# tsurumeso/vocal-remover

Measured on NVIDIA H100. Metric: seconds-of-audio/sec separated (n_fft=2048, hop=1024), higher is better.
Workload: dtype bf16x3 (split-bf16 operands hi+lo, 3 wgmma passes, fp32 accumulate); fft/lstm fp32

## Files before the change

vocal-remover_b200/csrc/api.cu:

```cuda
#include <stdio.h>
#include <string.h>

#include <string>

#include "../../include/vr_b200.h"
#include "engine.h"
#include "kernels.h"
#include "tc_plan.h"

struct vr_ctx {
  vr::Engine* eng;
  std::string err;
};

static std::string g_create_err;

static int fail(vr_ctx* c, const std::string& m) {
  (c ? c->err : g_create_err) = m;
  return -1;
}
static void use_device(const vr_ctx* c) {
  if (c && c->eng) cudaSetDevice(c->eng->cfg().device);
}
static int done(vr_ctx* c, bool ok) {
// ... 259 lines not shown
int vr_flac_encode_analyse(vr_ctx* ctx, const float* x, int32_t channels, int64_t n, int32_t rate_code, int32_t bits,
                           void* pcm, int32_t* plan, void* stream) {
  use_device(ctx);
  return cuda_result(ctx, "vr_flac_encode_analyse",
                     vr::launch_flac_encode_analyse(x, channels, n, rate_code, bits, pcm, plan, (cudaStream_t)stream));
}

int vr_flac_encode_pack(vr_ctx* ctx, const void* pcm, int32_t channels, int64_t n, int32_t bits, const int32_t* plan,
                        const int64_t* offsets, int32_t rate_code, int32_t rate_value, uint8_t* out, int32_t* status,
                        void* stream) {
  use_device(ctx);
  return cuda_result(ctx, "vr_flac_encode_pack",
                     vr::launch_flac_encode_pack(pcm, channels, n, bits, plan, offsets, rate_code, rate_value, out,
                                                 status, (cudaStream_t)stream));
}

int vr_pcm_pack(vr_ctx* ctx, const float* x, int32_t channels, int64_t n, int32_t bits, uint8_t* out, void* stream) {
  use_device(ctx);
  return cuda_result(ctx, "vr_pcm_pack", vr::launch_pcm_pack(x, channels, n, bits, out, (cudaStream_t)stream));
}

static int64_t bss_workspace(bool framewise, int32_t K, int32_t C, int64_t N, int32_t L, int64_t window, int64_t hop,
                             int32_t frames_per_batch) {
  std::string err;
  const int64_t bytes = vr::bss_eval_workspace(framewise, K, C, N, L, window, hop, frames_per_batch, err);
  if (bytes < 0) fail(nullptr, err);
  return bytes;
}

static int bss_run(vr_ctx* ctx, bool framewise, const float* refs, const float* ests, int32_t K, int32_t C, int64_t N,
                   int32_t L, int64_t window, int64_t hop, int32_t frames_per_batch, void* workspace,
                   int64_t workspace_bytes, double* frames_host, double* corr_host, double* loading_host,
                   double* phase_ms, void* stream) {
  use_device(ctx);
  std::string err;
  return vr::bss_eval(framewise, refs, ests, K, C, N, L, window, hop, frames_per_batch, workspace, workspace_bytes,
                      frames_host, corr_host, loading_host, phase_ms, (cudaStream_t)stream, err)
             ? 0
             : fail(ctx, err);
}

int64_t vr_bss_eval_workspace(int32_t K, int32_t C, int64_t N, int32_t L, int64_t window, int64_t hop) {
  return bss_workspace(false, K, C, N, L, window, hop, 1);
}

int vr_bss_eval(vr_ctx* ctx, const float* refs, const float* ests, int32_t K, int32_t C, int64_t N, int32_t L,
                int64_t window, int64_t hop, void* workspace, int64_t workspace_bytes, double* frames_host,
                double* corr_host, double* loading_host, double* phase_ms, void* stream) {
  return bss_run(ctx, false, refs, ests, K, C, N, L, window, hop, 1, workspace, workspace_bytes, frames_host,
                 corr_host, loading_host, phase_ms, stream);
}

int64_t vr_bss_eval_framewise_workspace(int32_t K, int32_t C, int64_t N, int32_t L, int64_t window, int64_t hop,
                                        int32_t frames_per_batch) {
  return bss_workspace(true, K, C, N, L, window, hop, frames_per_batch);
}

int vr_bss_eval_framewise(vr_ctx* ctx, const float* refs, const float* ests, int32_t K, int32_t C, int64_t N,
                          int32_t L, int64_t window, int64_t hop, int32_t frames_per_batch, void* workspace,
                          int64_t workspace_bytes, double* frames_host, double* corr_host, double* loading_host,
                          double* phase_ms, void* stream) {
  return bss_run(ctx, true, refs, ests, K, C, N, L, window, hop, frames_per_batch, workspace, workspace_bytes,
                 frames_host, corr_host, loading_host, phase_ms, stream);
}

int vr_shared_alloc(vr_ctx* ctx, int64_t bytes, void** dev_ptr, unsigned char* handle64) {
  CHECK_CTX(ctx);
  if (!dev_ptr || !handle64 || bytes <= 0) return fail(ctx, "vr_shared_alloc: bad arguments");
  static_assert(sizeof(cudaIpcMemHandle_t) == 64, "CUDA IPC handle is 64 bytes");
  void* p = nullptr;
  cudaError_t e = cudaMalloc(&p, (size_t)bytes);
  if (e != cudaSuccess) return fail(ctx, std::string("vr_shared_alloc: cudaMalloc: ") + cudaGetErrorString(e));
  cudaIpcMemHandle_t h;
  e = cudaIpcGetMemHandle(&h, p);
  if (e != cudaSuccess) {
    cudaFree(p);
    return fail(ctx, std::string("vr_shared_alloc: cudaIpcGetMemHandle: ") + cudaGetErrorString(e));
  }
  memcpy(handle64, &h, 64);
  *dev_ptr = p;
  return 0;
}

int vr_shared_open(vr_ctx* ctx, const unsigned char* handle64, void** dev_ptr) {
  CHECK_CTX(ctx);
  if (!dev_ptr || !handle64) return fail(ctx, "vr_shared_open: bad arguments");
  cudaIpcMemHandle_t h;
  memcpy(&h, handle64, 64);
  void* p = nullptr;
  cudaError_t e = cudaIpcOpenMemHandle(&p, h, cudaIpcMemLazyEnablePeerAccess);
  if (e != cudaSuccess) return fail(ctx, std::string("vr_shared_open: cudaIpcOpenMemHandle: ") + cudaGetErrorString(e));
  *dev_ptr = p;
  return 0;
}

int vr_shared_close(vr_ctx* ctx, void* dev_ptr, int32_t owner) {
  CHECK_CTX(ctx);
  if (!dev_ptr) return 0;
  cudaError_t e = owner ? cudaFree(dev_ptr) : cudaIpcCloseMemHandle(dev_ptr);
  if (e != cudaSuccess) return fail(ctx, std::string("vr_shared_close: ") + cudaGetErrorString(e));
  return 0;
}

int64_t vr_launch_count(const vr_ctx* ctx) { return ctx && ctx->eng ? ctx->eng->launches : 0; }

int vr_profile_enable(vr_ctx* ctx, int32_t on) {
  CHECK_CTX(ctx);
  ctx->eng->profile_enable(on != 0);
  return 0;
}

int vr_profile_read(vr_ctx* ctx, double* out6) {
  CHECK_CTX(ctx);
  return done(ctx, ctx->eng->profile_read(out6));
}

int vr_profile_dump(vr_ctx* ctx, char* text, int64_t cap, int64_t* needed) {
  CHECK_CTX(ctx);
  std::string t;
  if (!ctx->eng->profile_dump(t)) return done(ctx, false);
  if (needed) *needed = (int64_t)t.size() + 1;
  if (text && cap > 0) {
    const size_t n = t.size() < (size_t)cap - 1 ? t.size() : (size_t)cap - 1;
    memcpy(text, t.data(), n);
    text[n] = 0;
  }
  return 0;
}

int vr_debug_conv(vr_ctx* ctx, const float* x, int32_t N, int32_t Cin, int32_t H, int32_t W, const float* w,
                  const float* bias, int32_t Cout, int32_t k, int32_t stride, int32_t dil_h, int32_t dil_w, int32_t act,
                  int32_t use_tc, float* y, void* stream) {
  CHECK_CTX(ctx);
  return done(ctx, ctx->eng->debug_conv(x, N, Cin, H, W, w, bias, Cout, k, stride, dil_h, dil_w, act, use_tc, y,
                                        (cudaStream_t)stream));
}

int vr_debug_decoder(vr_ctx* ctx, const float* low, int32_t N, int32_t Cl, int32_t h, int32_t w, const float* skip,
                     int32_t Cs, const float* wgt, const float* bias, int32_t Cout, int32_t act, int32_t fused, float* y,
                     void* stream) {
  CHECK_CTX(ctx);
  return done(ctx, ctx->eng->debug_decoder(low, N, Cl, h, w, skip, Cs, wgt, bias, Cout, act, fused, y,
                                           (cudaStream_t)stream));
}

int vr_debug_tensor(vr_ctx* ctx, const char* name, int32_t n0, int32_t n, float* out, int64_t* shape4, void* stream) {
  CHECK_NET(ctx);
  if (!name || !shape4) return fail(ctx, "vr_debug_tensor: name and shape4 are required");
  return done(ctx, ctx->eng->debug_tensor(name, n0, n, out, shape4, (cudaStream_t)stream));
}

int vr_debug_set(int32_t key, int32_t value) {
  int* knob = key == 0 ? &vr::g_debug.trace : key == 2 ? &vr::g_debug.rows_wide : key == 3 ? &vr::g_debug.halo
            : key == 6 ? &vr::g_debug.kskip : key == 7 ? &vr::g_debug.crop_mask : nullptr;
  if (!knob) return -1;
  *knob = value;
  return 0;
}

int64_t vr_debug_trace(uint64_t* host_out, int64_t capacity) {
  return vr::tc_rows_read_trace((unsigned long long*)host_out, (long long)capacity);
}

}
```

vocal-remover_b200/csrc/conv_tc.cu:

```cuda
#include <cuda.h>
#include <stdio.h>

#include <map>
#include <tuple>

#include "engine.h"
#include "tc_common.cuh"
#include "tc_plan.h"

namespace vr {

static constexpr int kMaxStages = 8;
static constexpr int kConsumerWarps = 8;
static constexpr int kThreads = 32 * kConsumerWarps + 32;
static constexpr int kStaticSmem = 2048;

struct TcParams {
  int N, Ho, Wo, Wt, Ht, Nt, tiles_w, tiles_h, m_tiles, n_tiles;
  int stride, pad_h, pad_w, dil_h, dil_w, KW;
  int cchunks, total_sub, CinPadTC, Cout, act, stages;
  bf16* out_hi;
  bf16* out_lo;
  int64_t osn, osh;
  int osw;
  const float* bias;
};

template <int KB, int BN>
__global__ void __launch_bounds__(kThreads, 1)
    conv_tc_kernel(const __grid_constant__ CUtensorMap tmA, const __grid_constant__ CUtensorMap tmB, const TcParams p) {
  constexpr int SUBS = 64 / KB;
  constexpr int kSteps = KB / 16;
  constexpr uint32_t kAPlane = 128 * KB * 2;
  constexpr uint32_t kASub = 2 * kAPlane;
  constexpr uint32_t kBPlane = BN * KB * 2;
  constexpr uint32_t kBSub = 2 * kBPlane;
  constexpr uint32_t kStageBytes = SUBS * (kASub + kBSub);
  constexpr uint32_t kBRegion = SUBS * kASub;
  constexpr uint32_t kLayout = KB == 64 ? 1u : KB == 32 ? 2u : 3u;
  extern __shared__ uint8_t smem_raw[];
  __shared__ __align__(8) uint64_t bar_full[kMaxStages];
  __shared__ __align__(8) uint64_t bar_empty[kMaxStages];
  __shared__ float bias_s[256];

  const int warp = __shfl_sync(0xffffffffu, (int)threadIdx.x >> 5, 0);
  const int lane = threadIdx.x & 31;
  const uint32_t smem_base = (smem_u32(smem_raw) + 1023u) & ~1023u;
  const int total_tiles = p.m_tiles * p.n_tiles;
  const int num_iters = (p.total_sub + SUBS - 1) / SUBS;

  if (warp == kConsumerWarps && lane == 0) {
    tma_prefetch(&tmA);
    tma_prefetch(&tmB);
    MbarRing(smem_u32(&bar_full[0]), smem_u32(&bar_empty[0]), 0, p.stages).init(1, kConsumerWarps);
    asm volatile("fence.mbarrier_init.release.cluster;" ::: "memory");
  }
  for (int i = threadIdx.x; i < p.n_tiles * BN; i += blockDim.x) bias_s[i] = __ldg(p.bias + i);
  __syncthreads();

  if (warp == kConsumerWarps) {
    if (elect_one_sync()) {
      MbarRing ring(smem_u32(&bar_full[0]), smem_u32(&bar_empty[0]), 0, p.stages);
      for (int tile = blockIdx.x; tile < total_tiles; tile += gridDim.x) {
        const int nt = tile % p.n_tiles;
        const int mt = tile / p.n_tiles;
        const int w0 = (mt % p.tiles_w) * p.Wt;
        const int h0 = ((mt / p.tiles_w) % p.tiles_h) * p.Ht;
        const int n0 = (mt / (p.tiles_w * p.tiles_h)) * p.Nt;
        const int wbase = w0 * p.stride - p.pad_w, hbase = h0 * p.stride - p.pad_h;
        const int nrow = nt * BN;
        int cc = 0, kw = 0, kh = 0, sub = 0;
        for (int it = 0; it < num_iters; ++it) {
          ring.wait_empty();
          const int nsub = min(SUBS, p.total_sub - sub);
          const uint32_t full = ring.full();
          const uint32_t sbase = smem_base + (uint32_t)ring.slot * kStageBytes;
          mbar_expect_tx(full, (uint32_t)nsub * (kASub + kBSub));
#pragma unroll
          for (int j = 0; j < SUBS; ++j) {
            if (j < nsub) {
              tma_load_5d(sbase + (uint32_t)j * kASub, &tmA, cc * KB, wbase + kw * p.dil_w, hbase + kh * p.dil_h, n0, 0, full);
              tma_load_3d(sbase + kBRegion + (uint32_t)j * kBSub, &tmB, (kh * p.KW + kw) * p.CinPadTC + cc * KB, nrow, 0,
                          full);
              ++sub;
              if (++cc == p.cchunks) {
                cc = 0;
                if (++kw == p.KW) {
                  kw = 0;
                  ++kh;
                }
              }
            }
          }
          ring.advance();
        }
      }
    }
    __syncwarp();
  } else {
    const int wg = warp >> 2;
    const float slope = act_slope(p.act);
    const uint32_t dhi = desc_hi(8 * KB * 2, kLayout);
    MbarRing ring(smem_u32(&bar_full[0]), smem_u32(&bar_empty[0]), 0, p.stages);
    float acc[BN / 2];
    for (int tile = blockIdx.x; tile < total_tiles; tile += gridDim.x) {
#pragma unroll
      for (int i = 0; i < BN / 2; ++i) acc[i] = 0.f;
      HeldSlot held;
      for (int it = 0; it < num_iters; ++it) {
        const int nsub = min(SUBS, p.total_sub - it * SUBS);
        ring.wait_full();
        const uint32_t sdesc = desc_lo(smem_base + (uint32_t)ring.slot * kStageBytes);
        wg_fence();
#pragma unroll
        for (int j = 0; j < SUBS; ++j) {
          if (j < nsub) {
            const uint32_t a_hi = sdesc + ((j * kASub + (uint32_t)wg * (kAPlane / 2)) >> 4);
            const uint32_t a_lo = a_hi + (kAPlane >> 4);
            const uint32_t b_hi = sdesc + ((kBRegion + j * kBSub) >> 4);
            const uint32_t b_lo = b_hi + (kBPlane >> 4);
#pragma unroll
            for (int k = 0; k < kSteps; ++k)
              wgmma_split3<BN>(acc, a_hi + 2u * k, a_lo + 2u * k, b_hi + 2u * k, b_lo + 2u * k, dhi);
          }
        }
        wg_commit();
        wg_wait<1>();
        held.release(ring, lane);
        held.hold(ring);
        ring.advance();
      }
      wg_wait<0>();
      held.release_last(ring, lane);

      const int nt = tile % p.n_tiles;
      const int mt = tile / p.n_tiles;
      const int w0 = (mt % p.tiles_w) * p.Wt;
      const int h0 = ((mt / p.tiles_w) % p.tiles_h) * p.Ht;
      const int n0 = (mt / (p.tiles_w * p.tiles_h)) * p.Nt;
      const int c_lane = nt * BN + 2 * (lane & 3);
#pragma unroll
      for (int hr = 0; hr < 2; ++hr) {
        const int row = 64 * wg + 16 * (warp & 3) + (lane >> 2) + 8 * hr;
        const int dw = row % p.Wt;
        const int dh = (row / p.Wt) % p.Ht;
        const int n = n0 + row / (p.Wt * p.Ht);
        if (n >= p.N) continue;
        const int64_t obase = (int64_t)n * p.osn + (int64_t)(h0 + dh) * p.osh + (int64_t)(w0 + dw) * p.osw;
#pragma unroll
        for (int j = 0; j < BN / 8; ++j)
          epilogue_pair(acc[4 * j + 2 * hr], acc[4 * j + 2 * hr + 1], bias_s, c_lane + 8 * j, p.Cout, slope,
                        p.out_hi + obase, p.out_lo + obase);
      }
    }
  }
}

#define VR_TC_FOR_BN(X, KB) X(KB, 16) X(KB, 32) X(KB, 48) X(KB, 64) X(KB, 80) X(KB, 96) X(KB, 112) X(KB, 128)
#define VR_TC_FOR_ALL(X) VR_TC_FOR_BN(X, 64) VR_TC_FOR_BN(X, 32) VR_TC_FOR_BN(X, 16)


TcDebug g_debug;

static constexpr int kMaxDevices = 64;
const TcDevice& tc_device() {
  static TcDevice table[kMaxDevices];
  static TcDevice none;
  int dev = -1;
  if (cudaGetDevice(&dev) != cudaSuccess || dev < 0 || dev >= kMaxDevices) return none;
  TcDevice& d = table[dev];
  if (!d.ok) {
    if (cudaDeviceGetAttribute(&d.max_smem, cudaDevAttrMaxSharedMemoryPerBlockOptin, dev) != cudaSuccess ||
        cudaDeviceGetAttribute(&d.num_sms, cudaDevAttrMultiProcessorCount, dev) != cudaSuccess)
      return none;
#define VR_TC_SET_SMEM(KB, BN) \
  cudaFuncSetAttribute(conv_tc_kernel<KB, BN>, cudaFuncAttributeMaxDynamicSharedMemorySize, d.max_smem - kStaticSmem);
    VR_TC_FOR_ALL(VR_TC_SET_SMEM)
#undef VR_TC_SET_SMEM
    tc_rows_set_attributes(d.max_smem);
    tc_halo_set_attributes(d.max_smem);
    d.ok = true;
  }
  return d;
}

typedef CUresult (*EncodeTiledFn)(CUtensorMap*, CUtensorMapDataType, cuuint32_t, void*, const cuuint64_t*,
                                  const cuuint64_t*, const cuuint32_t*, const cuuint32_t*, CUtensorMapInterleave,
                                  CUtensorMapSwizzle, CUtensorMapL2promotion, CUtensorMapFloatOOBfill);
static EncodeTiledFn tc_encode_fn() {
  static EncodeTiledFn fn = nullptr;
  if (!fn) {
    void* p = nullptr;
    cudaDriverEntryPointQueryResult q;
    if (cudaGetDriverEntryPoint("cuTensorMapEncodeTiled", &p, cudaEnableDefault, &q) == cudaSuccess &&
        q == cudaDriverEntryPointSuccess)
      fn = (EncodeTiledFn)p;
  }
  return fn;
}

static CUtensorMapSwizzle swizzle_for(int KB) {
  return KB == 64 ? CU_TENSOR_MAP_SWIZZLE_128B : KB == 32 ? CU_TENSOR_MAP_SWIZZLE_64B : CU_TENSOR_MAP_SWIZZLE_32B;
}

static uint16_t tc_f2bf(float f) {
  uint32_t u;
  memcpy(&u, &f, 4);
  if ((u & 0x7fffffffu) > 0x7f800000u) return (uint16_t)((u >> 16) | 0x40);
  uint32_t r = 0x7fffu + ((u >> 16) & 1u);
  return (uint16_t)((u + r) >> 16);
}
static float tc_bf2f(uint16_t h) {
  uint32_t u = (uint32_t)h << 16;
  float f;
  memcpy(&f, &u, 4);
  return f;
}

struct TileGeom {
  int Wt, Ht, Nt;
  bool ok;
};
static TileGeom tile_geom(int Ho, int Wo) {
  TileGeom g{0, 0, 0, false};
  if (Wo <= 0 || Ho <= 0) return g;
  if (Wo >= 128) {
    if (Wo % 128) return g;
    g.Wt = 128; g.Ht = 1; g.Nt = 1;
  } else {
    if (128 % Wo) return g;
    g.Wt = Wo;
    g.Ht = 128 / Wo < Ho ? 128 / Wo : Ho;
    if (Ho % g.Ht) return g;
    if ((128 / Wo) % g.Ht) return g;
    g.Nt = 128 / (g.Wt * g.Ht);
  }
  g.ok = true;
  return g;
}

struct NTiling {
  int BN, n_tiles;
};
static NTiling n_tiling(const ConvLayer& L, bool rows, bool rows_wide) {
  const int cout16 = round_up(L.Cout, 16);
  if (rows) {
    const int BN = cout16 == 16 ? 16 : (rows_wide && cout16 % 64 == 0 ? 64 : 32);
    return {BN, ceil_div(cout16, BN)};
  }
  const int n_tiles = ceil_div(cout16, 128);
  return {round_up(ceil_div(cout16, n_tiles), 16), n_tiles};
}

TcKind tc_choose(const ConvLayer& L, int H, int W, bool rows_wide) {
  if (!(L.k == 1 || L.k == 3) || !(L.stride == 1 || L.stride == 2) || L.Cout < 4) return TC_NONE;
  const TileGeom g = tile_geom(H, W);
  if (!g.ok || g.Wt * L.stride > 256 || g.Ht * L.stride > 256) return TC_NONE;
  const bool k3s1 = L.k == 3 && L.stride == 1 && L.dil_h == 1 && L.dil_w == 1;
  const NTiling r = n_tiling(L, true, rows_wide), t = n_tiling(L, false, false);
  if (k3s1 && W % 128 == 0 && H % 8 == 0 && tc_rows_has(r.BN) && r.n_tiles * r.BN <= 256) return TC_ROWS;
  if (k3s1 && (W == 16 || W == 32 || W == 64) && H % (128 / W) == 0 && tc_halo_has(t.BN) &&
      t.n_tiles * t.BN <= 256 && g_debug.halo != 1)
    return TC_HALO;
  if (t.n_tiles * t.BN > 256) return TC_NONE;
  return TC_GENERIC;
}

template <class At>
static std::vector<uint16_t> split_bf16(const ConvLayer& L, const float* wp, int rows, int K, At at) {
  std::vector<uint16_t> planes((size_t)2 * rows * K, 0);
  const size_t lo = (size_t)rows * K;
  for (int co = 0; co < L.Cout; ++co)
    for (int t = 0; t < L.k * L.k; ++t)
      for (int ci = 0; ci < L.CinPad; ++ci) {
        const float w = wp[((size_t)t * L.CinPad + ci) * L.CoutPad + co];
        const uint16_t hi = tc_f2bf(w);
        const size_t i = at(co, t, ci);
        planes[i] = hi;
        planes[lo + i] = tc_f2bf(w - tc_bf2f(hi));
      }
  return planes;
}

static unsigned long long weight_group_mask(const ConvLayer& L, const float* wp, int CinPad) {
  if (CinPad / 8 > 64) return ~0ull;
  unsigned long long m = 0x3ull;
  for (int ci = 0; ci < L.CinPad; ++ci) {
    bool any = false;
    for (int t = 0; t < L.k * L.k && !any; ++t)
      for (int co = 0; co < L.Cout && !any; ++co) any = wp[((size_t)t * L.CinPad + ci) * L.CoutPad + co] != 0.f;
    if (any) m |= 1ull << (ci / 8);
  }
  return m;
}

static bool encode_weight_map(TcConv& tc, int rows, int K, int box_rows, std::string& err, const std::string& name) {
  cuuint64_t dims[3] = {(cuuint64_t)K, (cuuint64_t)rows, 2};
  cuuint64_t strides[2] = {(cuuint64_t)K * 2, (cuuint64_t)rows * K * 2};
  cuuint32_t box[3] = {(cuuint32_t)tc.KB, (cuuint32_t)box_rows, 2};
  cuuint32_t es[3] = {1, 1, 1};
  CUresult r = tc_encode_fn()(&tc.map_b, CU_TENSOR_MAP_DATA_TYPE_BFLOAT16, 3, tc.w_planes.get(), dims, strides, box, es,
                              CU_TENSOR_MAP_INTERLEAVE_NONE, swizzle_for(tc.KB), CU_TENSOR_MAP_L2_PROMOTION_L2_256B,
                              CU_TENSOR_MAP_FLOAT_OOB_FILL_NONE);
  if (r != CUDA_SUCCESS) {
    err = "cuTensorMapEncodeTiled(weights) failed for " + name + " code " + std::to_string((int)r);
    return false;
  }
  return true;
}

const CUtensorMap* tc_activation_map(TcConv& tc, const ActView& v, int bw, int bh, int bn, int es, std::string& err,
                                     const std::string& name) {
  const ViewKey key = std::make_tuple((const void*)v.hi, (const void*)v.lo, v.N, v.H, v.W, v.C, bw, bh, bn);
  auto it = tc.map_a.find(key);
  if (it != tc.map_a.end()) return &it->second;
  const int64_t plane = (const char*)v.lo - (const char*)v.hi;
  if (v.sw % 8 || v.sh % 8 || v.sn % 8 || (reinterpret_cast<uintptr_t>(v.hi) & 15) || plane <= 0 || plane % 16) {
    err = "internal: the input of " + name + " is not 16-byte aligned or its lo plane does not follow its hi plane";
    return nullptr;
  }
  cuuint64_t dims[5] = {(cuuint64_t)v.C, (cuuint64_t)v.W, (cuuint64_t)v.H, (cuuint64_t)v.N, 2};
  cuuint64_t strides[4] = {(cuuint64_t)v.sw * 2, (cuuint64_t)v.sh * 2, (cuuint64_t)v.sn * 2, (cuuint64_t)plane};
  cuuint32_t box[5] = {(cuuint32_t)tc.KB, (cuuint32_t)bw, (cuuint32_t)bh, (cuuint32_t)bn, 2};
  cuuint32_t estr[5] = {1, (cuuint32_t)es, (cuuint32_t)es, 1, 1};
  CUtensorMap m;
  CUresult r = tc_encode_fn()(&m, CU_TENSOR_MAP_DATA_TYPE_BFLOAT16, 5, (void*)v.hi, dims, strides, box, estr,
                              CU_TENSOR_MAP_INTERLEAVE_NONE, swizzle_for(tc.KB), CU_TENSOR_MAP_L2_PROMOTION_L2_256B,
                              CU_TENSOR_MAP_FLOAT_OOB_FILL_NONE);
  if (r != CUDA_SUCCESS) {
    err = "cuTensorMapEncodeTiled(activations) failed for " + name + " code " + std::to_string((int)r);
    return nullptr;
  }
  return &tc.map_a.emplace(key, m).first->second;
}

bool tc_prepare(ConvLayer& L, const float* w, const float* b, int H, int W, bool rows_wide, std::string& err) {
  const TcKind kind = tc_choose(L, H, W, rows_wide);
  if (kind == TC_NONE) return true;
  if (!tc_encode_fn()) {
    err = "cuTensorMapEncodeTiled is not available from the driver";
    return false;
  }
  auto tc = std::make_shared<TcConv>();
  tc->kind = kind;
  tc->H = H; tc->W = W;
  const NTiling nt = n_tiling(L, kind == TC_ROWS, rows_wide);
  const int BN = nt.BN, cin16 = round_up(L.CinPad, 16);
  tc->BN = BN; tc->n_tiles = nt.n_tiles;
  tc->KB = kind != TC_GENERIC ? 32 : cin16 % 64 == 0 ? 64 : cin16 % 32 == 0 ? 32 : 16;
  const int CinPad = round_up(L.CinPad, tc->KB);
  tc->CinPad = CinPad;
  tc->chunks = CinPad / tc->KB;
  tc->kmask = weight_group_mask(L, w, CinPad);
  const int rows = nt.n_tiles * BN;
  std::vector<uint16_t> planes;
  int brows, K;
  if (kind == TC_ROWS) {
    brows = 3 * rows;
    K = 3 * CinPad;
    planes = split_bf16(L, w, brows, K, [&](int co, int t, int ci) {
      return (size_t)(co / BN * 3 * BN + (2 - t / 3) * BN + co % BN) * K + (size_t)(t % 3) * CinPad + ci;
    });
  } else {
    brows = rows;
    K = L.k * L.k * CinPad;
    planes = split_bf16(L, w, brows, K, [&](int co, int t, int ci) { return (size_t)co * K + (size_t)t * CinPad + ci; });
  }
  std::vector<float> bias((size_t)rows, 0.f);
  for (int co = 0; co < L.Cout; ++co) bias[(size_t)co] = b[co];
  if (tc->w_planes.alloc(planes.size() * 2) != cudaSuccess || tc->bias.alloc(bias.size() * 4) != cudaSuccess) {
    err = "cudaMalloc failed while packing tensor-core weights for " + L.name;
    return false;
  }
  if (!upload(tc->w_planes.get(), planes.data(), planes.size() * 2, err) ||
      !upload(tc->bias.get(), bias.data(), bias.size() * 4, err) ||
      !encode_weight_map(*tc, brows, K, kind == TC_ROWS ? 3 * BN : BN, err, L.name))
    return false;
  L.tc = tc;
  return true;
}

cudaError_t tc_launch(const ConvLayer& L, const ActView& in, const ActView& out, cudaStream_t s, std::string& err,
                      const ConvFusion& f) {
  TcConv& tc = *L.tc;
  if (out.H != tc.H || out.W != tc.W || (in.H - 1) / L.stride + 1 != out.H || (in.W - 1) / L.stride + 1 != out.W) {
    err = "internal: " + L.name + " is launched on maps of another size than it was prepared for";
    return cudaErrorInvalidValue;
  }
  if (tc.kind == TC_ROWS) return tc_rows_launch(L, tc, in, out, s, err, f);
  if (!f.empty()) {
    err = "tc_launch: fused work is only implemented in the row-streaming kernel";
    return cudaErrorInvalidValue;
  }
  if (tc.kind == TC_HALO) return tc_halo_launch(L, tc, in, out, s, err);
  const TileGeom g = tile_geom(out.H, out.W);
  const CUtensorMap* map_a = tc_activation_map(tc, in, g.Wt * L.stride, g.Ht * L.stride, g.Nt, L.stride, err, L.name);
  if (!map_a) return cudaErrorInvalidValue;
  const int SUBS = 64 / tc.KB;
  TcParams p;
  p.N = out.N; p.Ho = out.H; p.Wo = out.W;
  p.Wt = g.Wt; p.Ht = g.Ht; p.Nt = g.Nt;
  p.tiles_w = out.W / g.Wt; p.tiles_h = out.H / g.Ht;
  p.m_tiles = p.tiles_w * p.tiles_h * ceil_div(out.N, g.Nt);
  p.n_tiles = tc.n_tiles;
  p.stride = L.stride; p.dil_h = L.dil_h; p.dil_w = L.dil_w;
  p.pad_h = L.dil_h * (L.k / 2); p.pad_w = L.dil_w * (L.k / 2);
  p.KW = L.k;
  p.cchunks = tc.chunks; p.total_sub = L.k * L.k * tc.chunks;
  p.CinPadTC = tc.CinPad; p.Cout = L.Cout; p.act = L.act;
  const int stage_bytes = SUBS * (2 * 128 * tc.KB * 2 + 2 * tc.BN * tc.KB * 2);
  const TcDevice& dv = tc_device();
  if (!dv.ok) {
    err = "tc_launch: cannot query the current device";
    return cudaErrorInvalidValue;
  }
  const int dyn = dv.max_smem - kStaticSmem;
  p.stages = (dyn - 1024) / stage_bytes;
  if (p.stages > kMaxStages) p.stages = kMaxStages;
  if (p.stages < 2) {
    err = "tc_launch: shared memory too small for two pipeline stages";
    return cudaErrorInvalidValue;
  }
  p.out_hi = out.hi; p.out_lo = out.lo;
  p.osn = out.sn; p.osh = out.sh; p.osw = out.sw;
  p.bias = tc.bias.get();
  const int total_tiles = p.m_tiles * p.n_tiles;
  const int grid = total_tiles < dv.num_sms ? total_tiles : dv.num_sms;
#define VR_TC_LAUNCH(KB_, BN_)                                                       \
  if (tc.KB == KB_ && tc.BN == BN_) {                                                \
    conv_tc_kernel<KB_, BN_><<<grid, kThreads, dyn, s>>>(*map_a, tc.map_b, p);       \
    return cudaGetLastError();                                                       \
  }
  VR_TC_FOR_ALL(VR_TC_LAUNCH)
#undef VR_TC_LAUNCH
  err = "tc_launch: no kernel instantiation for this channel tile";
  return cudaErrorInvalidValue;
}

}
```

vocal-remover_b200/csrc/tc_plan.h:

```cpp
#pragma once
#include <cuda.h>

#include <map>
#include <tuple>

#include "engine.h"

namespace vr {

enum TcKind {
  TC_NONE,
  TC_GENERIC,
  TC_ROWS,
  TC_HALO,
};

typedef std::tuple<const void*, const void*, int, int, int, int, int, int, int> ViewKey;

struct TcConv {
  TcKind kind = TC_NONE;
  int H = 0, W = 0;
  int KB = 0, CinPad = 0, chunks = 0, BN = 0, n_tiles = 0;
  unsigned long long kmask = ~0ull;
  DevPtr<bf16> w_planes;
  DevPtr<float> bias;
  CUtensorMap map_b;
  std::map<ViewKey, CUtensorMap> map_a;
  bool fuses_upsample(int up_C) const { return kind == TC_ROWS && up_C % 32 == 0 && up_C <= CinPad; }
  bool fuses_dot() const { return kind == TC_ROWS; }
  bool fuses_mask(int Cout, int offset, bool up) const {
    const int kept = W - 2 * offset;
    return kind == TC_ROWS && up && n_tiles == 1 && BN <= 32 && BN == Cout && offset >= 0 && kept > 0 &&
           kept % 128 == 0;
  }
};

TcKind tc_choose(const ConvLayer& L, int H, int W, bool rows_wide);
const CUtensorMap* tc_activation_map(TcConv& tc, const ActView& v, int bw, int bh, int bn, int es, std::string& err,
                                     const std::string& name);

cudaError_t tc_rows_launch(const ConvLayer& L, TcConv& tc, const ActView& in, const ActView& out, cudaStream_t s,
                           std::string& err, const ConvFusion& f);
void tc_rows_set_attributes(int max_smem);
bool tc_rows_has(int BN);
int tc_rows_read_trace(unsigned long long* out, long long capacity);

cudaError_t tc_halo_launch(const ConvLayer& L, TcConv& tc, const ActView& in, const ActView& out, cudaStream_t s,
                           std::string& err);
void tc_halo_set_attributes(int max_smem);
bool tc_halo_has(int BN);

struct TcDevice {
  bool ok = false;
  int num_sms = 0, max_smem = 0;
};
const TcDevice& tc_device();

struct TcDebug {
  int trace = 0;
  int rows_wide = 0;
  int halo = 0;
  int kskip = 1;
  int crop_mask = 1;
};
extern TcDebug g_debug;

}
```

Before: 2902.

## Pair M or N tiles per CTA in generic TC conv to share operand loads

Adds PAIR_M and PAIR_N modes to the generic tensor-core conv kernel. In these modes one CTA runs 16 consumer warps over two M tiles that share a B tile, or two N tiles that share an A tile, with a smaller K stage. A heuristic picks pairing only for small KB/BN layers, and only when it cuts the number of SM waves roughly in half. The goal is to reduce redundant operand traffic and wave quantization on small layers. The epilogue also gains vectorized 16-byte stores, at the cost of more template instantiations, extra tensor maps and higher register pressure.

```diff
diff --git a/profiles/generic_conv.py b/profiles/generic_conv.py
--- /dev/null
+++ b/profiles/generic_conv.py
@@ -0,0 +1,171 @@
+import argparse
+import ctypes
+import json
+import os
+import statistics
+import subprocess
+import sys
+
+ROOT = os.path.dirname(os.path.dirname(os.path.abspath(__file__)))
+PKG = os.path.join(ROOT, 'vocal-remover_b200')
+for p in (ROOT, PKG):
+    if p not in sys.path:
+        sys.path.insert(0, p)
+
+NETS = [('stg1_low', 16, 512), ('stg1_high', 8, 512), ('stg2_low', 32, 512), ('stg2_high', 16, 512),
+        ('stg3_full', 32, 1024)]
+W = 256
+NOUT = 32
+
+
+def generic_layers():
+    out = {}
+    mult = [1, 2, 4, 6, 8]
+    for net, n, H in NETS:
+        for i in range(4):
+            key = (n * mult[i], H >> i, W >> i, n * mult[i + 1], 3, 2, 1, 1, 2)
+            out.setdefault(key, []).append('%s.enc%d.conv1' % (net, i + 2))
+        c8, h16, w16 = 8 * n, H // 16, W // 16
+        out.setdefault((c8, 1, w16, c8, 1, 1, 1, 1, 1), []).append(net + '.aspp.conv1.1')
+        out.setdefault((c8, h16, w16, c8, 1, 1, 1, 1, 1), []).append(net + '.aspp.conv2')
+        for j, (dh, dw) in enumerate([(4, 2), (8, 4), (12, 6)]):
+            out.setdefault((c8, h16, w16, c8, 3, 1, dh, dw, 1), []).append('%s.aspp.conv%d' % (net, j + 3))
+        out.setdefault((5 * c8, h16, w16, c8, 1, 1, 1, 1, 1), []).append(net + '.aspp.bottleneck')
+    out.setdefault((NOUT // 2, 512, W, NOUT // 4, 1, 1, 1, 1, 1), []).append('stg1_low_band_net.1')
+    out.setdefault((NOUT, 512, W, NOUT // 2, 1, 1, 1, 1, 1), []).append('stg2_low_band_net.1')
+    return out
+
+
+def _ceil(a, b):
+    return -(-a // b)
+
+
+def tiling(N, g):
+    Cin, H, Wi, Cout, k, s = g[:6]
+    Ho, Wo = (H - 1) // s + 1, (Wi - 1) // s + 1
+    cout16 = _ceil(Cout, 16) * 16
+    n_tiles = _ceil(cout16, 128)
+    BN = _ceil(_ceil(cout16, n_tiles), 16) * 16
+    cin16 = _ceil(Cin, 16) * 16
+    if Wo >= 128:
+        Wt, Ht, Nt = 128, 1, 1
+    else:
+        Wt, Ht = Wo, min(128 // Wo, Ho)
+        Nt = 128 // (Wt * Ht)
+    m_tiles = (Wo // Wt) * (Ho // Ht) * _ceil(N, Nt)
+    KB = 64 if cin16 % 64 == 0 else 32 if cin16 % 32 == 0 else 16
+    return dict(Ho=Ho, Wo=Wo, BN=BN, n_tiles=n_tiles, m_tiles=m_tiles, CinPad=cin16, KB=KB,
+                flops=2.0 * N * Ho * Wo * Cout * Cin * k * k)
+
+
+def operand_bytes(t, k, mode):
+    per = k * k * t['CinPad'] * 4
+    m, nt, BN = t['m_tiles'], t['n_tiles'], t['BN']
+    if mode == 'PAIR_M':
+        return per * nt * (128 * m + BN * _ceil(m, 2))
+    if mode == 'PAIR_N':
+        return per * m * (128 + 2 * BN)
+    return per * m * nt * (128 + BN)
+
+
+def auto_mode(t, num_sms):
+    if t['KB'] > 32 or t['BN'] > 32:
+        return 'NONE'
+    pair = 'PAIR_N' if t['n_tiles'] == 2 and t['KB'] >= 32 else 'PAIR_M'
+    units = t['m_tiles'] if pair == 'PAIR_N' else _ceil(t['m_tiles'], 2) * t['n_tiles']
+    w1, w2 = _ceil(t['m_tiles'] * t['n_tiles'], num_sms), _ceil(units, num_sms)
+    return pair if 19 * w2 <= 10 * w1 else 'NONE'
+
+
+def _gpu_info():
+    try:
+        r = subprocess.run(['nvidia-smi', '--query-gpu=name,power.limit,clocks.max.sm,clocks.sm',
+                            '--format=csv,noheader'], capture_output=True, text=True, timeout=30)
+        name, power, max_clock, clock = [s.strip() for s in r.stdout.splitlines()[0].split(',')]
+        return dict(gpu=name, power_limit=power, max_sm_clock=max_clock, sm_clock=clock)
+    except Exception as e:
+        return dict(gpu=None, nvidia_smi_error=str(e))
+
+
+def _run_conv(ctx, x, w, b, g):
+    import torch
+    from lib import _native
+    Cin, H, Wi, Cout, k, s, dh, dw, act = g
+    N = x.shape[0]
+    Ho, Wo = (H - 1) // s + 1, (Wi - 1) // s + 1
+    y = torch.empty((N, Cout, Ho, Wo), dtype=torch.float32, device='cuda')
+    ctx.check(ctx.lib.vr_debug_conv(ctx.handle, _native.ptr(x), N, Cin, H, Wi, _native.ptr(w), _native.ptr(b), Cout,
+                                    k, s, dh, dw, act, 1, _native.ptr(y), _native.stream_ptr()), 'vr_debug_conv')
+
+
+def _profiled_ms(ctx):
+    need = ctypes.c_int64(0)
+    ctx.check(ctx.lib.vr_profile_dump(ctx.handle, None, 0, ctypes.byref(need)), 'vr_profile_dump')
+    buf = ctypes.create_string_buffer(need.value)
+    ctx.check(ctx.lib.vr_profile_dump(ctx.handle, buf, need.value, None), 'vr_profile_dump')
+    return [float(ln.split()[5]) for ln in buf.value.decode().splitlines() if ln.split()[0] == 'debug_conv']
+
+
+def main():
+    ap = argparse.ArgumentParser()
+    ap.add_argument('--batch', type=int, default=27)
+    ap.add_argument('--runs', type=int, default=10)
+    ap.add_argument('--warmup', type=int, default=3)
+    ap.add_argument('--out', type=str, default='')
+    args = ap.parse_args()
+    import torch
+    from lib import _native
+    assert torch.cuda.is_available(), 'generic_conv.py times the GPU kernels: it needs a CUDA device'
+    info = _gpu_info()
+    info['torch_device'] = torch.cuda.get_device_name(0)
+    num_sms = torch.cuda.get_device_properties(0).multi_processor_count
+    ctx = _native.Context(0, 2048, 1024, NOUT, 128, 256, 1, 0)
+    modes = [(1, 'NONE'), (2, 'PAIR_M'), (3, 'PAIR_N'), (0, 'auto')]
+    rows = []
+    N = args.batch
+    print('# %s, power limit %s, max SM clock %s (SM clock %s at start); batch %d, median of %d launches'
+          % (info.get('gpu') or info['torch_device'], info.get('power_limit'), info.get('max_sm_clock'),
+             info.get('sm_clock'), N, args.runs))
+    print('%-28s %-38s %5s %5s %6s  %-8s %8s %7s %8s' % ('layers', 'Cin,H,W,Cout,k,s,dh,dw', 'BN', 'nt', 'mt', 'key',
+                                                         'ms', 'TFLOP/s', 'B/FLOP'))
+    try:
+        for gi, (g, names) in enumerate(generic_layers().items()):
+            Cin, H, Wi, Cout, k = g[:5]
+            t = tiling(N, g)
+            gen = torch.Generator().manual_seed(gi)
+            x = torch.randn(N, Cin, H, Wi, generator=gen).cuda()
+            w = (torch.randn(Cout, Cin, k, k, generator=gen) / (Cin * k * k) ** 0.5).cuda()
+            b = (torch.randn(Cout, generator=gen) * 0.1).cuda()
+            auto = auto_mode(t, num_sms)
+            for key, mode in modes:
+                if mode == 'PAIR_N' and not (t['n_tiles'] == 2 and t['KB'] >= 32):
+                    continue
+                ctx.lib.vr_debug_set(8, key)
+                for _ in range(args.warmup):
+                    _run_conv(ctx, x, w, b, g)
+                ctx.check(ctx.lib.vr_profile_enable(ctx.handle, 1), 'vr_profile_enable')
+                for _ in range(args.runs):
+                    _run_conv(ctx, x, w, b, g)
+                ms = statistics.median(_profiled_ms(ctx))
+                ctx.check(ctx.lib.vr_profile_enable(ctx.handle, 0), 'vr_profile_enable')
+                ran = auto if mode == 'auto' else mode
+                bpf = operand_bytes(t, k, ran) / t['flops']
+                row = dict(layers=names, geometry=list(g), batch=N, key=key, mode=ran, ms=ms,
+                           tflops=t['flops'] / ms * 1e-9, operand_bytes_per_flop=bpf, **t)
+                rows.append(row)
+                print('%-28s %-38s %5d %5d %6d  %-8s %8.4f %7.1f %8.4f' % (
+                    names[0] + ('' if len(names) == 1 else ' +%d' % (len(names) - 1)), ','.join(map(str, g[:8])),
+                    t['BN'], t['n_tiles'], t['m_tiles'], '%d %s' % (key, ran if key == 0 else ''), ms,
+                    row['tflops'], bpf))
+    finally:
+        ctx.lib.vr_debug_set(8, 0)
+        ctx.close()
+    info_end = _gpu_info()
+    print('# SM clock at end: %s' % info_end.get('sm_clock'))
+    if args.out:
+        with open(args.out, 'w') as f:
+            json.dump(dict(gpu=info, sm_clock_end=info_end.get('sm_clock'), rows=rows), f, indent=1)
+
+
+if __name__ == '__main__':
+    main()
diff --git a/vocal-remover_b200/csrc/api.cu b/vocal-remover_b200/csrc/api.cu
--- a/vocal-remover_b200/csrc/api.cu
+++ b/vocal-remover_b200/csrc/api.cu
@@ -435,7 +435,8 @@
 
 int vr_debug_set(int32_t key, int32_t value) {
   int* knob = key == 0 ? &vr::g_debug.trace : key == 2 ? &vr::g_debug.rows_wide : key == 3 ? &vr::g_debug.halo
-            : key == 6 ? &vr::g_debug.kskip : key == 7 ? &vr::g_debug.crop_mask : nullptr;
+            : key == 6 ? &vr::g_debug.kskip : key == 7 ? &vr::g_debug.crop_mask
+            : key == 8 ? &vr::g_debug.pair : nullptr;
   if (!knob) return -1;
   *knob = value;
   return 0;
diff --git a/vocal-remover_b200/csrc/conv_tc.cu b/vocal-remover_b200/csrc/conv_tc.cu
--- a/vocal-remover_b200/csrc/conv_tc.cu
+++ b/vocal-remover_b200/csrc/conv_tc.cu
@@ -11,8 +11,9 @@
 namespace vr {
 
 static constexpr int kMaxStages = 8;
-static constexpr int kConsumerWarps = 8;
-static constexpr int kThreads = 32 * kConsumerWarps + 32;
+__host__ __device__ constexpr int consumer_warps(int mode) { return mode == PAIR_NONE ? 8 : 16; }
+__host__ __device__ constexpr int tc_threads(int mode) { return 32 * consumer_warps(mode) + 32; }
+__host__ __device__ constexpr int stage_k(int mode) { return mode == PAIR_NONE ? 64 : 32; }
 static constexpr int kStaticSmem = 2048;
 
 struct TcParams {
@@ -24,19 +25,33 @@
   int64_t osn, osh;
   int osw;
   const float* bias;
+  int vec16;
 };
 
-template <int KB, int BN>
-__global__ void __launch_bounds__(kThreads, 1)
+__device__ __forceinline__ void act_split2(float v0, float v1, const float* bias_s, int c, float slope, uint32_t& hi,
+                                           uint32_t& lo) {
+  const float t0 = v0 + bias_s[c], t1 = v1 + bias_s[c + 1];
+  const float y0 = fmaxf(t0, 0.f) + slope * fminf(t0, 0.f);
+  const float y1 = fmaxf(t1, 0.f) + slope * fminf(t1, 0.f);
+  hi = f2_to_bf2(y0, y1);
+  const float2 hf = bf2_to_f2(hi);
+  lo = f2_to_bf2(y0 - hf.x, y1 - hf.y);
+}
+
+template <int KB, int BN, int MODE>
+__global__ void __launch_bounds__(tc_threads(MODE), 1)
     conv_tc_kernel(const __grid_constant__ CUtensorMap tmA, const __grid_constant__ CUtensorMap tmB, const TcParams p) {
-  constexpr int SUBS = 64 / KB;
+  constexpr int kConsumerWarps = consumer_warps(MODE);
+  constexpr int SUBS = stage_k(MODE) / KB;
+  constexpr int NA = MODE == PAIR_M ? 2 : 1;
+  constexpr int NB = MODE == PAIR_N ? 2 : 1;
   constexpr int kSteps = KB / 16;
   constexpr uint32_t kAPlane = 128 * KB * 2;
   constexpr uint32_t kASub = 2 * kAPlane;
   constexpr uint32_t kBPlane = BN * KB * 2;
   constexpr uint32_t kBSub = 2 * kBPlane;
-  constexpr uint32_t kStageBytes = SUBS * (kASub + kBSub);
-  constexpr uint32_t kBRegion = SUBS * kASub;
+  constexpr uint32_t kStageBytes = SUBS * (NA * kASub + NB * kBSub);
+  constexpr uint32_t kBRegion = SUBS * NA * kASub;
   constexpr uint32_t kLayout = KB == 64 ? 1u : KB == 32 ? 2u : 3u;
   extern __shared__ uint8_t smem_raw[];
   __shared__ __align__(8) uint64_t bar_full[kMaxStages];
@@ -46,7 +61,8 @@
   const int warp = __shfl_sync(0xffffffffu, (int)threadIdx.x >> 5, 0);
   const int lane = threadIdx.x & 31;
   const uint32_t smem_base = (smem_u32(smem_raw) + 1023u) & ~1023u;
-  const int total_tiles = p.m_tiles * p.n_tiles;
+  const int n_units = p.n_tiles / NB;
+  const int total_units = (p.m_tiles + NA - 1) / NA * n_units;
   const int num_iters = (p.total_sub + SUBS - 1) / SUBS;
 
   if (warp == kConsumerWarps && lane == 0) {
@@ -61,27 +77,37 @@
   if (warp == kConsumerWarps) {
     if (elect_one_sync()) {
       MbarRing ring(smem_u32(&bar_full[0]), smem_u32(&bar_empty[0]), 0, p.stages);
-      for (int tile = blockIdx.x; tile < total_tiles; tile += gridDim.x) {
-        const int nt = tile % p.n_tiles;
-        const int mt = tile / p.n_tiles;
-        const int w0 = (mt % p.tiles_w) * p.Wt;
-        const int h0 = ((mt / p.tiles_w) % p.tiles_h) * p.Ht;
-        const int n0 = (mt / (p.tiles_w * p.tiles_h)) * p.Nt;
-        const int wbase = w0 * p.stride - p.pad_w, hbase = h0 * p.stride - p.pad_h;
-        const int nrow = nt * BN;
+      for (int unit = blockIdx.x; unit < total_units; unit += gridDim.x) {
+        const int nt0 = unit % n_units * NB;
+        const int mt0 = unit / n_units * NA;
+        const int na = min(NA, p.m_tiles - mt0);
+        int wbase[NA], hbase[NA], n0[NA];
+#pragma unroll
+        for (int a = 0; a < NA; ++a) {
+          const int mt = mt0 + a;
+          wbase[a] = (mt % p.tiles_w) * p.Wt * p.stride - p.pad_w;
+          hbase[a] = ((mt / p.tiles_w) % p.tiles_h) * p.Ht * p.stride - p.pad_h;
+          n0[a] = (mt / (p.tiles_w * p.tiles_h)) * p.Nt;
+        }
         int cc = 0, kw = 0, kh = 0, sub = 0;
         for (int it = 0; it < num_iters; ++it) {
           ring.wait_empty();
           const int nsub = min(SUBS, p.total_sub - sub);
           const uint32_t full = ring.full();
           const uint32_t sbase = smem_base + (uint32_t)ring.slot * kStageBytes;
-          mbar_expect_tx(full, (uint32_t)nsub * (kASub + kBSub));
+          mbar_expect_tx(full, (uint32_t)nsub * ((uint32_t)na * kASub + NB * kBSub));
 #pragma unroll
           for (int j = 0; j < SUBS; ++j) {
             if (j < nsub) {
-              tma_load_5d(sbase + (uint32_t)j * kASub, &tmA, cc * KB, wbase + kw * p.dil_w, hbase + kh * p.dil_h, n0, 0, full);
-              tma_load_3d(sbase + kBRegion + (uint32_t)j * kBSub, &tmB, (kh * p.KW + kw) * p.CinPadTC + cc * KB, nrow, 0,
-                          full);
+#pragma unroll
+              for (int a = 0; a < NA; ++a)
+                if (a < na)
+                  tma_load_5d(sbase + (uint32_t)(j * NA + a) * kASub, &tmA, cc * KB, wbase[a] + kw * p.dil_w,
+                              hbase[a] + kh * p.dil_h, n0[a], 0, full);
+#pragma unroll
+              for (int b = 0; b < NB; ++b)
+                tma_load_3d(sbase + kBRegion + (uint32_t)(j * NB + b) * kBSub, &tmB,
+                            (kh * p.KW + kw) * p.CinPadTC + cc * KB, (nt0 + b) * BN, 0, full);
               ++sub;
               if (++cc == p.cchunks) {
                 cc = 0;
@@ -98,12 +124,24 @@
     }
     __syncwarp();
   } else {
-    const int wg = warp >> 2;
+    const int half = (warp >> 2) & 1;
+    const int pair = warp >> 3;
+    const int a_sel = MODE == PAIR_M ? pair : 0, b_sel = MODE == PAIR_N ? pair : 0;
     const float slope = act_slope(p.act);
     const uint32_t dhi = desc_hi(8 * KB * 2, kLayout);
     MbarRing ring(smem_u32(&bar_full[0]), smem_u32(&bar_empty[0]), 0, p.stages);
     float acc[BN / 2];
-    for (int tile = blockIdx.x; tile < total_tiles; tile += gridDim.x) {
+    for (int unit = blockIdx.x; unit < total_units; unit += gridDim.x) {
+      const int nt = unit % n_units * NB + b_sel;
+      const int mt = unit / n_units * NA + a_sel;
+      if (mt >= p.m_tiles) {
+        for (int it = 0; it < num_iters; ++it) {
+          ring.wait_full();
+          warp_arrive(ring.empty(), lane);
+          ring.advance();
+        }
+        continue;
+      }
 #pragma unroll
       for (int i = 0; i < BN / 2; ++i) acc[i] = 0.f;
       HeldSlot held;
@@ -115,9 +153,9 @@
 #pragma unroll
         for (int j = 0; j < SUBS; ++j) {
           if (j < nsub) {
-            const uint32_t a_hi = sdesc + ((j * kASub + (uint32_t)wg * (kAPlane / 2)) >> 4);
+            const uint32_t a_hi = sdesc + (((j * NA + a_sel) * kASub + (uint32_t)half * (kAPlane / 2)) >> 4);
             const uint32_t a_lo = a_hi + (kAPlane >> 4);
-            const uint32_t b_hi = sdesc + ((kBRegion + j * kBSub) >> 4);
+            const uint32_t b_hi = sdesc + ((kBRegion + (j * NB + b_sel) * kBSub) >> 4);
             const uint32_t b_lo = b_hi + (kBPlane >> 4);
 #pragma unroll
             for (int k = 0; k < kSteps; ++k)
@@ -133,31 +171,72 @@
       wg_wait<0>();
       held.release_last(ring, lane);
 
-      const int nt = tile % p.n_tiles;
-      const int mt = tile / p.n_tiles;
       const int w0 = (mt % p.tiles_w) * p.Wt;
       const int h0 = ((mt / p.tiles_w) % p.tiles_h) * p.Ht;
       const int n0 = (mt / (p.tiles_w * p.tiles_h)) * p.Nt;
-      const int c_lane = nt * BN + 2 * (lane & 3);
+      const int q = lane & 3;
+      const int c_lane = nt * BN + 2 * q;
 #pragma unroll
       for (int hr = 0; hr < 2; ++hr) {
-        const int row = 64 * wg + 16 * (warp & 3) + (lane >> 2) + 8 * hr;
+        const int row = 64 * half + 16 * (warp & 3) + (lane >> 2) + 8 * hr;
         const int dw = row % p.Wt;
         const int dh = (row / p.Wt) % p.Ht;
         const int n = n0 + row / (p.Wt * p.Ht);
-        if (n >= p.N) continue;
         const int64_t obase = (int64_t)n * p.osn + (int64_t)(h0 + dh) * p.osh + (int64_t)(w0 + dw) * p.osw;
-#pragma unroll
-        for (int j = 0; j < BN / 8; ++j)
-          epilogue_pair(acc[4 * j + 2 * hr], acc[4 * j + 2 * hr + 1], bias_s, c_lane + 8 * j, p.Cout, slope,
-                        p.out_hi + obase, p.out_lo + obase);
+        if constexpr (BN % 32 == 0 && (MODE == PAIR_NONE || BN <= 64)) {
+          const bool keep = n < p.N;
+#pragma unroll
+          for (int jb = 0; jb < BN / 8; jb += 4) {
+            if (p.vec16 && nt * BN + 8 * (jb + 4) <= p.Cout) {
+              uint32_t hi[4], lo[4], oh[4], ol[4];
+#pragma unroll
+              for (int g = 0; g < 4; ++g)
+                act_split2(acc[4 * (jb + g) + 2 * hr], acc[4 * (jb + g) + 2 * hr + 1], bias_s, c_lane + 8 * (jb + g),
+                           slope, hi[g], lo[g]);
+#pragma unroll
+              for (int s = 0; s < 4; ++s) {
+                const int gs = (q + s) & 3, src = (q - s) & 3;
+                const uint32_t sh = gs == 0 ? hi[0] : gs == 1 ? hi[1] : gs == 2 ? hi[2] : hi[3];
+                const uint32_t sl = gs == 0 ? lo[0] : gs == 1 ? lo[1] : gs == 2 ? lo[2] : lo[3];
+                const uint32_t rh = __shfl_sync(0xffffffffu, sh, (lane & ~3) | src);
+                const uint32_t rl = __shfl_sync(0xffffffffu, sl, (lane & ~3) | src);
+#pragma unroll
+                for (int g = 0; g < 4; ++g)
+                  if (src == g) {
+                    oh[g] = rh;
+                    ol[g] = rl;
+                  }
+              }
+              if (keep) {
+                const int c = nt * BN + 8 * (jb + q);
+                *reinterpret_cast<uint4*>(p.out_hi + obase + c) = make_uint4(oh[0], oh[1], oh[2], oh[3]);
+                *reinterpret_cast<uint4*>(p.out_lo + obase + c) = make_uint4(ol[0], ol[1], ol[2], ol[3]);
+              }
+            } else if (keep) {
+#pragma unroll
+              for (int j = jb; j < jb + 4; ++j)
+                epilogue_pair(acc[4 * j + 2 * hr], acc[4 * j + 2 * hr + 1], bias_s, c_lane + 8 * j, p.Cout, slope,
+                              p.out_hi + obase, p.out_lo + obase);
+            }
+          }
+        } else {
+          if (n >= p.N) continue;
+#pragma unroll
+          for (int j = 0; j < BN / 8; ++j)
+            epilogue_pair(acc[4 * j + 2 * hr], acc[4 * j + 2 * hr + 1], bias_s, c_lane + 8 * j, p.Cout, slope,
+                          p.out_hi + obase, p.out_lo + obase);
+        }
       }
     }
   }
 }
 
-#define VR_TC_FOR_BN(X, KB) X(KB, 16) X(KB, 32) X(KB, 48) X(KB, 64) X(KB, 80) X(KB, 96) X(KB, 112) X(KB, 128)
-#define VR_TC_FOR_ALL(X) VR_TC_FOR_BN(X, 64) VR_TC_FOR_BN(X, 32) VR_TC_FOR_BN(X, 16)
+#define VR_TC_FOR_BN(X, KB, M) \
+  X(KB, 16, M) X(KB, 32, M) X(KB, 48, M) X(KB, 64, M) X(KB, 80, M) X(KB, 96, M) X(KB, 112, M) X(KB, 128, M)
+#define VR_TC_FOR_ALL(X)                                                                                   \
+  VR_TC_FOR_BN(X, 64, PAIR_NONE) VR_TC_FOR_BN(X, 32, PAIR_NONE) VR_TC_FOR_BN(X, 16, PAIR_NONE)             \
+  VR_TC_FOR_BN(X, 32, PAIR_M) VR_TC_FOR_BN(X, 16, PAIR_M)                                                  \
+  X(32, 80, PAIR_N) X(32, 96, PAIR_N) X(32, 112, PAIR_N) X(32, 128, PAIR_N)
 
 
 TcDebug g_debug;
@@ -173,8 +252,8 @@
     if (cudaDeviceGetAttribute(&d.max_smem, cudaDevAttrMaxSharedMemoryPerBlockOptin, dev) != cudaSuccess ||
         cudaDeviceGetAttribute(&d.num_sms, cudaDevAttrMultiProcessorCount, dev) != cudaSuccess)
       return none;
-#define VR_TC_SET_SMEM(KB, BN) \
-  cudaFuncSetAttribute(conv_tc_kernel<KB, BN>, cudaFuncAttributeMaxDynamicSharedMemorySize, d.max_smem - kStaticSmem);
+#define VR_TC_SET_SMEM(KB, BN, M) \
+  cudaFuncSetAttribute(conv_tc_kernel<KB, BN, M>, cudaFuncAttributeMaxDynamicSharedMemorySize, d.max_smem - kStaticSmem);
     VR_TC_FOR_ALL(VR_TC_SET_SMEM)
 #undef VR_TC_SET_SMEM
     tc_rows_set_attributes(d.max_smem);
@@ -294,13 +373,14 @@
   return m;
 }
 
-static bool encode_weight_map(TcConv& tc, int rows, int K, int box_rows, std::string& err, const std::string& name) {
+static bool encode_weight_map(const TcConv& tc, CUtensorMap* map, int kb, int rows, int K, int box_rows,
+                              std::string& err, const std::string& name) {
   cuuint64_t dims[3] = {(cuuint64_t)K, (cuuint64_t)rows, 2};
   cuuint64_t strides[2] = {(cuuint64_t)K * 2, (cuuint64_t)rows * K * 2};
-  cuuint32_t box[3] = {(cuuint32_t)tc.KB, (cuuint32_t)box_rows, 2};
+  cuuint32_t box[3] = {(cuuint32_t)kb, (cuuint32_t)box_rows, 2};
   cuuint32_t es[3] = {1, 1, 1};
-  CUresult r = tc_encode_fn()(&tc.map_b, CU_TENSOR_MAP_DATA_TYPE_BFLOAT16, 3, tc.w_planes.get(), dims, strides, box, es,
-                              CU_TENSOR_MAP_INTERLEAVE_NONE, swizzle_for(tc.KB), CU_TENSOR_MAP_L2_PROMOTION_L2_256B,
+  CUresult r = tc_encode_fn()(map, CU_TENSOR_MAP_DATA_TYPE_BFLOAT16, 3, tc.w_planes.get(), dims, strides, box, es,
+                              CU_TENSOR_MAP_INTERLEAVE_NONE, swizzle_for(kb), CU_TENSOR_MAP_L2_PROMOTION_L2_256B,
                               CU_TENSOR_MAP_FLOAT_OOB_FILL_NONE);
   if (r != CUDA_SUCCESS) {
     err = "cuTensorMapEncodeTiled(weights) failed for " + name + " code " + std::to_string((int)r);
@@ -310,8 +390,9 @@
 }
 
 const CUtensorMap* tc_activation_map(TcConv& tc, const ActView& v, int bw, int bh, int bn, int es, std::string& err,
-                                     const std::string& name) {
-  const ViewKey key = std::make_tuple((const void*)v.hi, (const void*)v.lo, v.N, v.H, v.W, v.C, bw, bh, bn);
+                                     const std::string& name, int kb) {
+  if (kb == 0) kb = tc.KB;
+  const ViewKey key = std::make_tuple((const void*)v.hi, (const void*)v.lo, v.N, v.H, v.W, v.C, bw, bh, bn, kb);
   auto it = tc.map_a.find(key);
   if (it != tc.map_a.end()) return &it->second;
   const int64_t plane = (const char*)v.lo - (const char*)v.hi;
@@ -321,11 +402,11 @@
   }
   cuuint64_t dims[5] = {(cuuint64_t)v.C, (cuuint64_t)v.W, (cuuint64_t)v.H, (cuuint64_t)v.N, 2};
   cuuint64_t strides[4] = {(cuuint64_t)v.sw * 2, (cuuint64_t)v.sh * 2, (cuuint64_t)v.sn * 2, (cuuint64_t)plane};
-  cuuint32_t box[5] = {(cuuint32_t)tc.KB, (cuuint32_t)bw, (cuuint32_t)bh, (cuuint32_t)bn, 2};
+  cuuint32_t box[5] = {(cuuint32_t)kb, (cuuint32_t)bw, (cuuint32_t)bh, (cuuint32_t)bn, 2};
   cuuint32_t estr[5] = {1, (cuuint32_t)es, (cuuint32_t)es, 1, 1};
   CUtensorMap m;
   CUresult r = tc_encode_fn()(&m, CU_TENSOR_MAP_DATA_TYPE_BFLOAT16, 5, (void*)v.hi, dims, strides, box, estr,
-                              CU_TENSOR_MAP_INTERLEAVE_NONE, swizzle_for(tc.KB), CU_TENSOR_MAP_L2_PROMOTION_L2_256B,
+                              CU_TENSOR_MAP_INTERLEAVE_NONE, swizzle_for(kb), CU_TENSOR_MAP_L2_PROMOTION_L2_256B,
                               CU_TENSOR_MAP_FLOAT_OOB_FILL_NONE);
   if (r != CUDA_SUCCESS) {
     err = "cuTensorMapEncodeTiled(activations) failed for " + name + " code " + std::to_string((int)r);
@@ -374,10 +455,25 @@
   }
   if (!upload(tc->w_planes.get(), planes.data(), planes.size() * 2, err) ||
       !upload(tc->bias.get(), bias.data(), bias.size() * 4, err) ||
-      !encode_weight_map(*tc, brows, K, kind == TC_ROWS ? 3 * BN : BN, err, L.name))
+      !encode_weight_map(*tc, &tc->map_b, tc->KB, brows, K, kind == TC_ROWS ? 3 * BN : BN, err, L.name))
     return false;
+  if (kind == TC_GENERIC) {
+    tc->pair_KB = tc->KB < 32 ? tc->KB : 32;
+    tc->pair = tc->n_tiles == 2 && tc->pair_KB == 32 ? PAIR_N : PAIR_M;
+    if (!encode_weight_map(*tc, &tc->map_b_pair, tc->pair_KB, brows, K, BN, err, L.name)) return false;
+  }
   L.tc = tc;
   return true;
+}
+
+static TcPair launch_pairing(const TcConv& tc, int m_tiles, int num_sms) {
+  if (g_debug.pair == 1) return PAIR_NONE;
+  if (g_debug.pair == 2) return PAIR_M;
+  if (g_debug.pair == 3) return tc.pair == PAIR_N ? PAIR_N : PAIR_NONE;
+  if (tc.KB > 32 || tc.BN > 32) return PAIR_NONE;
+  const int units = tc.pair == PAIR_N ? m_tiles : ceil_div(m_tiles, 2) * tc.n_tiles;
+  const int waves1 = ceil_div(m_tiles * tc.n_tiles, num_sms), waves2 = ceil_div(units, num_sms);
+  return 19 * waves2 <= 10 * waves1 ? tc.pair : PAIR_NONE;
 }
 
 cudaError_t tc_launch(const ConvLayer& L, const ActView& in, const ActView& out, cudaStream_t s, std::string& err,
@@ -393,10 +489,12 @@
     return cudaErrorInvalidValue;
   }
   if (tc.kind == TC_HALO) return tc_halo_launch(L, tc, in, out, s, err);
+  const TcDevice& dv = tc_device();
+  if (!dv.ok) {
+    err = "tc_launch: cannot query the current device";
+    return cudaErrorInvalidValue;
+  }
   const TileGeom g = tile_geom(out.H, out.W);
-  const CUtensorMap* map_a = tc_activation_map(tc, in, g.Wt * L.stride, g.Ht * L.stride, g.Nt, L.stride, err, L.name);
-  if (!map_a) return cudaErrorInvalidValue;
-  const int SUBS = 64 / tc.KB;
   TcParams p;
   p.N = out.N; p.Ho = out.H; p.Wo = out.W;
   p.Wt = g.Wt; p.Ht = g.Ht; p.Nt = g.Nt;
@@ -406,14 +504,15 @@
   p.stride = L.stride; p.dil_h = L.dil_h; p.dil_w = L.dil_w;
   p.pad_h = L.dil_h * (L.k / 2); p.pad_w = L.dil_w * (L.k / 2);
   p.KW = L.k;
-  p.cchunks = tc.chunks; p.total_sub = L.k * L.k * tc.chunks;
   p.CinPadTC = tc.CinPad; p.Cout = L.Cout; p.act = L.act;
-  const int stage_bytes = SUBS * (2 * 128 * tc.KB * 2 + 2 * tc.BN * tc.KB * 2);
-  const TcDevice& dv = tc_device();
-  if (!dv.ok) {
-    err = "tc_launch: cannot query the current device";
-    return cudaErrorInvalidValue;
-  }
+  const TcPair mode = launch_pairing(tc, p.m_tiles, dv.num_sms);
+  const int KB = mode == PAIR_NONE ? tc.KB : tc.pair_KB;
+  p.cchunks = tc.CinPad / KB; p.total_sub = L.k * L.k * p.cchunks;
+  const CUtensorMap* map_a = tc_activation_map(tc, in, g.Wt * L.stride, g.Ht * L.stride, g.Nt, L.stride, err, L.name, KB);
+  if (!map_a) return cudaErrorInvalidValue;
+  const CUtensorMap& map_b = mode == PAIR_NONE ? tc.map_b : tc.map_b_pair;
+  const int na = mode == PAIR_M ? 2 : 1, nb = mode == PAIR_N ? 2 : 1;
+  const int stage_bytes = stage_k(mode) / KB * (na * 2 * 128 * KB * 2 + nb * 2 * tc.BN * KB * 2);
   const int dyn = dv.max_smem - kStaticSmem;
   p.stages = (dyn - 1024) / stage_bytes;
   if (p.stages > kMaxStages) p.stages = kMaxStages;
@@ -423,13 +522,15 @@
   }
   p.out_hi = out.hi; p.out_lo = out.lo;
   p.osn = out.sn; p.osh = out.sh; p.osw = out.sw;
+  p.vec16 = ((reinterpret_cast<uintptr_t>(out.hi) | reinterpret_cast<uintptr_t>(out.lo)) & 15) == 0 && out.sn % 8 == 0 &&
+            out.sh % 8 == 0 && out.sw % 8 == 0;
   p.bias = tc.bias.get();
-  const int total_tiles = p.m_tiles * p.n_tiles;
-  const int grid = total_tiles < dv.num_sms ? total_tiles : dv.num_sms;
-#define VR_TC_LAUNCH(KB_, BN_)                                                       \
-  if (tc.KB == KB_ && tc.BN == BN_) {                                                \
-    conv_tc_kernel<KB_, BN_><<<grid, kThreads, dyn, s>>>(*map_a, tc.map_b, p);       \
-    return cudaGetLastError();                                                       \
+  const int total_units = ceil_div(p.m_tiles, na) * (p.n_tiles / nb);
+  const int grid = total_units < dv.num_sms ? total_units : dv.num_sms;
+#define VR_TC_LAUNCH(KB_, BN_, M_)                                                          \
+  if (KB == KB_ && tc.BN == BN_ && mode == M_) {                                            \
+    conv_tc_kernel<KB_, BN_, M_><<<grid, tc_threads(M_), dyn, s>>>(*map_a, map_b, p);       \
+    return cudaGetLastError();                                                              \
   }
   VR_TC_FOR_ALL(VR_TC_LAUNCH)
 #undef VR_TC_LAUNCH
diff --git a/vocal-remover_b200/csrc/tc_plan.h b/vocal-remover_b200/csrc/tc_plan.h
--- a/vocal-remover_b200/csrc/tc_plan.h
+++ b/vocal-remover_b200/csrc/tc_plan.h
@@ -15,7 +15,9 @@
   TC_HALO,
 };
 
-typedef std::tuple<const void*, const void*, int, int, int, int, int, int, int> ViewKey;
+enum TcPair { PAIR_NONE = 0, PAIR_M = 1, PAIR_N = 2 };
+
+typedef std::tuple<const void*, const void*, int, int, int, int, int, int, int, int> ViewKey;
 
 struct TcConv {
   TcKind kind = TC_NONE;
@@ -26,6 +28,9 @@
   DevPtr<float> bias;
   CUtensorMap map_b;
   std::map<ViewKey, CUtensorMap> map_a;
+  TcPair pair = PAIR_NONE;
+  int pair_KB = 0;
+  CUtensorMap map_b_pair;
   bool fuses_upsample(int up_C) const { return kind == TC_ROWS && up_C % 32 == 0 && up_C <= CinPad; }
   bool fuses_dot() const { return kind == TC_ROWS; }
   bool fuses_mask(int Cout, int offset, bool up) const {
@@ -37,7 +42,7 @@
 
 TcKind tc_choose(const ConvLayer& L, int H, int W, bool rows_wide);
 const CUtensorMap* tc_activation_map(TcConv& tc, const ActView& v, int bw, int bh, int bn, int es, std::string& err,
-                                     const std::string& name);
+                                     const std::string& name, int kb = 0);
 
 cudaError_t tc_rows_launch(const ConvLayer& L, TcConv& tc, const ActView& in, const ActView& out, cudaStream_t s,
                            std::string& err, const ConvFusion& f);
@@ -62,6 +67,7 @@
   int halo = 0;
   int kskip = 1;
   int crop_mask = 1;
+  int pair = 0;
 };
 extern TcDebug g_debug;
 
```

Result: faster. 2993, median of 6 (+3.1%).
